# MiRaCLeXeoN/sduss

Hardware: AMD Instinct MI355X
Metric: images/sec (node), SDXL 1024^2 50-step, fixed prompt, CFG (higher is better)
Workload: dtype bf16; 1 GPU; SDXL-base-1.0 UNet 1024x1024 50-step Euler, CFG 5.0, 4 requests/step (denoiser batch 8) per GPU, is_sliced=False, random-init weights of the real architecture (2.57 B params), one data-parallel replica per GPU, no collective; resolution=1024, steps_per_image=50

## Files before the change

### include/mxdenoise.h

```cpp
#ifndef MXDENOISE_H
#define MXDENOISE_H

#include <stddef.h>
#include <stdint.h>

#ifdef __cplusplus
extern "C" {
#endif

enum { MX_F32 = 0, MX_F16 = 1, MX_BF16 = 2 };

const char* mx_last_error(void);
int mx_version(void);
#define MX_PROF_KINDS 12
int mx_profile_enable(int on);
int mx_profile_collect(double* out);
int mx_profile_records(double* out, int max_records);

size_t mx_groupnorm_halo_workspace_bytes(int N, int C, int cpg);
int mx_groupnorm_halo(void* stream, const void* x, const void* gamma, const void* beta, void* y,
                      int N, int C, int H, int W, int cpg, double eps, int padding,
                      const int32_t* latent_offset, int n_latents, const int32_t* patch_map,
                      const int32_t* padding_idx, int dtype, void* workspace);
int mx_halo_only(void* stream, const void* x, void* y, int N, int C, int H, int W,
// ... 89 lines not shown
#define MX_STATS_PITCH(slabs) (((slabs) + 3) & ~3)
int mx_row_stats(void* stream, const void* x, int ldx, float* stats, int M, int C);
int mx_conv3x3(void* stream, const mx_gemm_desc* d);
int mx_gemm_splitk(const mx_gemm_desc* d, int conv);
void mx_gemm_release_scratch(void* stream, int all);

#define MX_VT_POS(key) (((key) & ~12) | (((key) & 4) << 1) | (((key) & 8) >> 1))
#define MX_VT_LD(Lk) (((Lk) + 15) / 16 * 16)

int mx_attention(void* stream, const void* q, int ldq, const void* k, int ldk, const void* vt, int ldvt,
                 int64_t vt_batch_stride, void* o, int ldo, int B, int H, int Lq, int Lk, float scale);
#define MX_ATTN_QSCALE(scale) ((scale) * 1.4426950408889634f)
int mx_attention_prescaled(void* stream, const void* q, int ldq, const void* k, int ldk, const void* vt, int ldvt,
                           int64_t vt_batch_stride, void* o, int ldo, int B, int H, int Lq, int Lk);
int mx_attention_cross_prescaled(void* stream, const void* q, int ldq, const void* k, int ldk, const void* vt, int ldvt,
                                 int64_t vt_batch_stride, void* o, int ldo, int B, int H, int Lq, int Lk);
typedef struct mx_attn_problem {
  const void* q; const void* k; const void* vt; void* o;
  int64_t vt_batch_stride;
  int B, Lq, Lk, ldvt;
} mx_attn_problem;
int mx_attention_prescaled_grouped(void* stream, const mx_attn_problem* probs, int n, int ldq, int ldk, int ldo, int H);
int mx_attention_prescaled_bias(void* stream, const void* q, int ldq, const void* k, int ldk, const void* vt, int ldvt,
                                int64_t vt_batch_stride, void* o, int ldo, int B, int H, int Lq, int Lk, const float* bias, int ldb);
int mx_attention_prescaled_causal(void* stream, const void* q, int ldq, const void* k, int ldk, const void* vt, int ldvt,
                                  int64_t vt_batch_stride, void* o, int ldo, int B, int H, int L);

int mx_layernorm(void* stream, const void* x, void* y, const float* gamma, const float* beta,
                 int M, int C, float eps);

int mx_rmsnorm(void* stream, const void* x, void* y, const float* w, int M, int C, float eps);

int mx_layernorm_mod(void* stream, const void* x, void* y, void* y2, const float* scale, const float* shift,
                     const float* scale2, const float* shift2, int ldmod, int M, int C, int rows_per_batch, float eps);
int mx_layernorm_mod_grouped(void* stream, const void* x, void* y, void* y2, const float* scale, const float* shift, const float* scale2,
                             const float* shift2, int ldmod, int C, float eps, const int* batches, const int* rows_per_batch, int n);
int mx_rmsnorm_heads(void* stream, void* x, int ld, int nbatch, int rows_per_batch, int batch_rows, int row_off,
                     int heads_total, int heads_q, const float* wq, const float* wk, float eps, float q_scale);

size_t mx_groupnorm_nhwc_workspace_bytes(int B, int H, int W, int C);
int mx_groupnorm_nhwc(void* stream, const void* x, void* y, const float* gamma, const float* beta,
                      int B, int H, int W, int C, int groups, float eps, int silu, int patch,
                      void* workspace);

int mx_groupnorm_nhwc_cat(void* stream, const void* x, int C1, const void* x2, void* y, const float* gamma, const float* beta,
                          int B, int H, int W, int C, int groups, float eps, int silu, int patch, void* workspace);
int mx_groupnorm_nhwc_from_partials(void* stream, const void* x, void* y, const float* gamma, const float* beta, int B, int H, int W, int C, int groups, float eps,
                                    int silu, const float* part, int chunk, const float* add_bias, const float* add_rowbias, int ldrb, void* workspace);

typedef struct mx_gn_problem { const void* x; const void* x2; void* y; int B, H, W; } mx_gn_problem;
size_t mx_groupnorm_nhwc_grouped_workspace_bytes(const mx_gn_problem* probs, int n, int C);
int mx_groupnorm_nhwc_grouped(void* stream, const mx_gn_problem* probs, int n, int C1, const float* gamma, const float* beta, int C, int groups,
                              float eps, int silu, int patch, void* workspace);

typedef struct mx_unet_config {
  int in_channels, out_channels;
  int n_levels;
  int block_out_channels[4];
  int layers_per_block;
  int down_has_attn[4];
  int transformer_layers[4];
  int num_heads[4];
  int cross_attention_dim;
  int addition_time_embed_dim;
  int projection_class_embeddings_input_dim;
  int norm_num_groups;
  float norm_eps, transformer_norm_eps, layer_norm_eps;
} mx_unet_config;

typedef struct mx_weight_entry {
  const char* name;
  uint64_t offset;
  uint64_t bytes;
} mx_weight_entry;

typedef struct mx_unet mx_unet;

mx_unet* mx_unet_create(const mx_unet_config* cfg);
void mx_unet_destroy(mx_unet* u);
int mx_unet_set_weights(mx_unet* u, const void* blob, uint64_t blob_bytes,
                        const mx_weight_entry* table, int n_entries);
int mx_unet_set_context_key(mx_unet* u, uint64_t key);
int mx_unet_context_stats(const mx_unet* u, long* hits, long* misses);
size_t mx_unet_workspace_bytes(const mx_unet* u, int batch, int H, int W, int ctx_len);
int mx_unet_validate(const mx_unet* u, int batch, int H, int W, int ctx_len);
int mx_unet_forward(mx_unet* u, void* stream, const void* latents, int io_dtype, const float* timesteps,
                    const void* ehs, const void* text_embeds, const float* time_ids, void* out,
                    int batch, int H, int W, int ctx_len, int gn_patch, void* workspace, size_t workspace_bytes);
typedef struct mx_unet_group { const void* latents; void* out; int batch, H, W; } mx_unet_group;
size_t mx_unet_workspace_bytes_mixed(const mx_unet* u, const mx_unet_group* groups, int n_groups, int ctx_len);
int mx_unet_forward_mixed(mx_unet* u, void* stream, const mx_unet_group* groups, int n_groups, int io_dtype, const float* timesteps,
                          const void* ehs, const void* text_embeds, const float* time_ids, int ctx_len, int gn_patch, void* workspace,
                          size_t workspace_bytes);
int mx_unet_forward_mixed_trace(mx_unet* u, void* stream, const mx_unet_group* groups, int n_groups, int io_dtype, const float* timesteps,
                                const void* ehs, const void* text_embeds, const float* time_ids, int ctx_len, int gn_patch, void* workspace,
                                size_t workspace_bytes, const char* stage, void* stage_out, size_t stage_out_bytes);
int mx_unet_forward_trace(mx_unet* u, void* stream, const void* latents, int io_dtype, const float* timesteps,
                          const void* ehs, const void* text_embeds, const float* time_ids, void* out,
                          int batch, int H, int W, int ctx_len, int gn_patch, void* workspace,
                          size_t workspace_bytes, const char* stage, void* stage_out, size_t stage_out_bytes);

typedef int (*mx_allgather_fn)(void* ctx, void* stream, const void* send, void* recv, size_t bytes_per_rank);
typedef struct mx_pp_comm { int rank, world; mx_allgather_fn all_gather; void* ctx; } mx_pp_comm;
size_t mx_unet_workspace_bytes_pp(const mx_unet* u, int batch, int H_local, int W, int ctx_len, int world);
int mx_unet_forward_pp(mx_unet* u, void* stream, const void* latents_local, int io_dtype, const float* timesteps, const void* ehs,
                       const void* text_embeds, const float* time_ids, void* out_local, int batch, int H_local, int W, int ctx_len,
// ... 209 lines not shown
```

### sduss_amd/csrc/norm.hip

```cpp
#include <cstdlib>

#include "common.h"
#include "../../include/mxdenoise.h"

namespace mx {

struct GnGeom {
  int B, H, W, C;
  int tpr;
  int L;
  int th, tw;
  int tiles_y, tiles_x;
  const bf16_t* x2;
  int C1;
};

struct GnProb {
  GnGeom g;
  const bf16_t* x; bf16_t* y;
  float* part; float* coef;
  float* gpart;
  long y_img;
  int ppb;
  int patch;
};
struct GnGroup {
  GnProb p[MX_MAX_SEGS];
  int blk0[MX_MAX_SEGS + 1];
  int n;
};
__device__ __forceinline__ const GnProb& gn_locate(const GnGroup& G, int& local) {
  local = blockIdx.x;
  int s = 0;
#pragma unroll
  for (int i = 1; i < MX_MAX_SEGS; ++i) if (i < G.n && local >= G.blk0[i]) s = i;
  local -= G.blk0[s];
  return G.p[s];
}

__device__ __forceinline__ const bf16_t* gn_src(const bf16_t* x, const GnGeom& g, long pix, int ch) {
  if (g.x2 == nullptr) return x + pix * g.C + ch;
  return ch < g.C1 ? x + pix * g.C1 + ch : g.x2 + pix * (g.C - g.C1) + (ch - g.C1);
}

__global__ void gn_stats_kernel(const GnGroup G, const int groups) {
  extern __shared__ __attribute__((aligned(16))) float red[];
  const int t = threadIdx.x;
  int local;
  const GnProb& P = gn_locate(G, local);
  const GnGeom& g = P.g;
  const bf16_t* __restrict__ x = P.x;
  float* __restrict__ part = P.part;
  const int ntl = g.tiles_y * g.tiles_x;
  const int b = local / ntl;
  const int tile = local - b * ntl;
  const int ty = tile / g.tiles_x, tx = tile - ty * g.tiles_x;
  const int cv = t % g.tpr;
  const int pl = t / g.tpr;
  float s[8], ss[8];
#pragma unroll
  for (int e = 0; e < 8; ++e) { s[e] = 0.f; ss[e] = 0.f; }
  if (pl < g.L) {
    const int npix = g.th * g.tw;
    for (int pi = pl; pi < npix; pi += g.L) {
      const int py = pi / g.tw, px = pi - py * g.tw;
      const long pix = ((long)b * g.H + ty * g.th + py) * g.W + tx * g.tw + px;
      const u32x4 v = *reinterpret_cast<const u32x4*>(gn_src(x, g, pix, cv * 8));
#pragma unroll
      for (int e = 0; e < 4; ++e) {
        const float lo = bf16lo_to_f32(v[e]), hi = bf16hi_to_f32(v[e]);
        s[2 * e] += lo; ss[2 * e] += lo * lo;
        s[2 * e + 1] += hi; ss[2 * e + 1] += hi * hi;
      }
    }
#pragma unroll
    for (int e = 0; e < 8; ++e) {
      red[((long)pl * g.C + cv * 8 + e) * 2] = s[e];
      red[((long)pl * g.C + cv * 8 + e) * 2 + 1] = ss[e];
    }
  }
  __syncthreads();
  float* __restrict__ gpart = P.gpart;
  float* chs = red + (long)g.L * g.C * 2;
  for (int c = t; c < g.C; c += blockDim.x) {
    float a = 0.f, q = 0.f;
    for (int l = 0; l < g.L; ++l) { a += red[((long)l * g.C + c) * 2]; q += red[((long)l * g.C + c) * 2 + 1]; }
    if (gpart != nullptr) { chs[2 * c] = a; chs[2 * c + 1] = q; continue; }
    float* dst = part + (((long)b * (g.tiles_y * g.tiles_x) + tile) * g.C + c) * 2;
    dst[0] = a; dst[1] = q;
  }
  if (gpart != nullptr) {
// ... 107 lines not shown
      double s = 0.0, q = 0.0;
      for (int tl = sub; tl < ntl; tl += 8) {
        const float2 v = *reinterpret_cast<const float2*>(gp + ((long)tl * groups + gi) * 2);
        s += (double)v.x; q += (double)v.y;
      }
      fsub[gi][sub][0] = s; fsub[gi][sub][1] = q;
    }
    __syncthreads();
    const int cpg = g.C / groups;
    const double cnt = (double)g.H * g.W * cpg;
    for (int gi = t; gi < groups; gi += blockDim.x) {
      double s = 0.0, q = 0.0;
#pragma unroll
      for (int sub = 0; sub < 8; ++sub) { s += fsub[gi][sub][0]; q += fsub[gi][sub][1]; }
      const double mean = s / cnt;
      double var = q / cnt - mean * mean;
      if (var < 0.0) var = 0.0;
      mr[gi][0] = mean;
      mr[gi][1] = 1.0 / sqrt(var + (double)eps);
    }
    __syncthreads();
    if (pl >= g.L) return;
#pragma unroll
    for (int e = 0; e < 8; ++e) {
      const int ch = cv * 8 + e;
      const int gi = ch / cpg;
      const double rg = mr[gi][1] * (double)gamma[ch];
      sc[e] = (float)rg;
      sf[e] = (float)((double)beta[ch] - rg * mr[gi][0]);
    }
  } else {
    if (pl >= g.L) return;
    const float* cf = coef + ((long)b * g.C + cv * 8) * 2;
#pragma unroll
    for (int e = 0; e < 8; ++e) { sc[e] = cf[2 * e]; sf[e] = cf[2 * e + 1]; }
  }
  const int hw = g.H * g.W;
  const int p0 = pblk * pix_per_block;
  const int p1 = min(p0 + pix_per_block, hw);
  for (int pi = p0 + pl; pi < p1; pi += g.L) {
    const u32x4 v = *reinterpret_cast<const u32x4*>(gn_src(x, g, (long)b * hw + pi, cv * 8));
    u32x4 o;
#pragma unroll
    for (int e = 0; e < 4; ++e) {
      float lo = bf16lo_to_f32(v[e]) * sc[2 * e] + sf[2 * e];
      float hi = bf16hi_to_f32(v[e]) * sc[2 * e + 1] + sf[2 * e + 1];
      if (SILU) { lo = silu_f(lo); hi = silu_f(hi); }
      o[e] = pack_bf16x2(lo, hi);
    }
    *reinterpret_cast<u32x4*>(y + (long)b * y_img + (long)pi * g.C + cv * 8) = o;
  }
}

__global__ __launch_bounds__(64) void gn_pp_sums_kernel(const float* __restrict__ part, double* __restrict__ sums, GnGeom g, int groups) {
  const int grp = blockIdx.x, b = blockIdx.y, lane = threadIdx.x;
  const int cpg = g.C / groups;
  const int ntiles = g.tiles_y * g.tiles_x;
  double s = 0.0, q = 0.0;
  for (int it = lane; it < ntiles * cpg; it += 64) {
    const int tile = it / cpg, c = it - tile * cpg;
    const float* src = part + (((long)b * ntiles + tile) * g.C + grp * cpg + c) * 2;
    s += (double)src[0];
    q += (double)src[1];
  }
  s = wave_sum_d(s);
  q = wave_sum_d(q);
  if (lane == 0) { sums[((long)b * groups + grp) * 2] = s; sums[((long)b * groups + grp) * 2 + 1] = q; }
}

__global__ __launch_bounds__(64) void gn_pp_coef_kernel(const double* __restrict__ all_sums, const float* __restrict__ gamma,
                                                        const float* __restrict__ beta, float* __restrict__ coef, int B, int C,
                                                        int groups, int world, double cnt, float eps,
                                                        const double* __restrict__ fresh_own, int own_rank) {
  const int grp = blockIdx.x, b = blockIdx.y, lane = threadIdx.x;
  const int cpg = C / groups;
  double s = 0.0, q = 0.0;
  for (int r = 0; r < world; ++r) {
    s += all_sums[(((long)r * B + b) * groups + grp) * 2];
    q += all_sums[(((long)r * B + b) * groups + grp) * 2 + 1];
  }
  double var_fallback = 0.0;
  if (fresh_own) {
    const long o = (((long)own_rank * B + b) * groups + grp) * 2, f = ((long)b * groups + grp) * 2;
    s += (double)world * (fresh_own[f] - all_sums[o]);
    q += (double)world * (fresh_own[f + 1] - all_sums[o + 1]);
    const double lc = cnt / world, lm = fresh_own[f] / lc;
    var_fallback = fresh_own[f + 1] / lc - lm * lm;
    if (var_fallback < 0.0) var_fallback = 0.0;
  }
  const double mean = s / cnt;
  double var = q / cnt - mean * mean;
  if (var < 0.0) var = var_fallback;
  const double rstd = 1.0 / sqrt(var + (double)eps);
  for (int c = lane; c < cpg; c += 64) {
    const int ch = grp * cpg + c;
    coef[((long)b * C + ch) * 2] = (float)(rstd * (double)gamma[ch]);
    coef[((long)b * C + ch) * 2 + 1] = (float)((double)beta[ch] - rstd * (double)gamma[ch] * mean);
  }
}

static int gn_geom(GnGeom& g, int B, int H, int W, int C, int patch) {
  MX_CHECK(C % 8 == 0 && C / 8 <= 1024, "groupnorm: C must be a multiple of 8 and <= 8192");
  g.B = B; g.H = H; g.W = W; g.C = C;
  g.x2 = nullptr; g.C1 = C;
  g.tpr = C / 8;
  g.L = 1024 / g.tpr;
// ... 32 lines not shown
  return mx_groupnorm_nhwc_cat(stream, x, C, nullptr, y, gamma, beta, B, H, W, C, groups, eps, silu, patch, workspace);
}

namespace mx {
static size_t gn_fill(GnGroup& G, int i, const void* x, int C1, const void* x2, void* y, long y_img, int B, int H, int W, int C, int patch, char* ws) {
  GnProb& P = G.p[i];
  if (patch >= H && patch >= W) patch = 0;
  if (patch != 0 && patch < 2) { set_error("groupnorm: patch must be 0 or >= 2"); return 0; }
  if (gn_geom(P.g, B, H, W, C, patch)) return 0;
  if (x2) { P.g.x2 = (const bf16_t*)x2; P.g.C1 = C1; }
  const size_t ntiles = (size_t)P.g.tiles_y * P.g.tiles_x;
  P.x = (const bf16_t*)x; P.y = (bf16_t*)y; P.y_img = y_img; P.patch = patch;
  P.part = (float*)ws;
  P.gpart = nullptr;
  P.coef = P.part + (size_t)B * ntiles * C * 2;
  const int hw = H * W;
  P.ppb = P.g.L * 8 > hw ? hw : P.g.L * 8;
  return (((size_t)B * ntiles * C * 2 + (size_t)B * C * 2) * sizeof(float) + 255) & ~(size_t)255;
}
static void gn_prefix(GnGroup& G, int which, int groups) {
  long t = 0;
  for (int i = 0; i < G.n; ++i) {
    G.blk0[i] = (int)t;
    const GnGeom& g = G.p[i].g;
    t += which == 0 ? (long)g.B * g.tiles_y * g.tiles_x : which == 1 ? (long)g.B * groups : (long)g.B * cdiv(g.H * g.W, G.p[i].ppb);
  }
  for (int i = G.n; i <= MX_MAX_SEGS; ++i) G.blk0[i] = (int)t;
}
static int gn_launch_stats(hipStream_t s, GnGroup& G, int C, int groups = 0) {
  const GnGeom& g = G.p[0].g;
  const int threads = ((g.tpr * g.L + 63) / 64) * 64;
  const size_t smem = ((size_t)g.L * C * 2 + (groups > 0 ? (size_t)C * 2 : 0)) * sizeof(float);
  MX_CHECK(smem <= 160 * 1024, "groupnorm: LDS budget exceeded");
  gn_prefix(G, 0, 0);
  hipLaunchKernelGGL(gn_stats_kernel, dim3(G.blk0[MX_MAX_SEGS]), dim3(threads), smem, s, G, groups);
  MX_LAUNCH_CHECK();
  return 0;
}
static int gn_launch_apply(hipStream_t s, GnGroup& G, int silu, bool fold = false, const float* gamma = nullptr, const float* beta = nullptr, int groups = 0, float eps = 0.f) {
  const GnGeom& g = G.p[0].g;
  const int threads = ((g.tpr * g.L + 63) / 64) * 64;
  gn_prefix(G, 2, 0);
  const dim3 grid(G.blk0[MX_MAX_SEGS]), block(threads);
  if (fold) {
    if (silu) hipLaunchKernelGGL((gn_apply_kernel<true, true>), grid, block, 0, s, G, gamma, beta, groups, eps);
    else hipLaunchKernelGGL((gn_apply_kernel<false, true>), grid, block, 0, s, G, gamma, beta, groups, eps);
  } else {
    if (silu) hipLaunchKernelGGL((gn_apply_kernel<true, false>), grid, block, 0, s, G, gamma, beta, groups, eps);
    else hipLaunchKernelGGL((gn_apply_kernel<false, false>), grid, block, 0, s, G, gamma, beta, groups, eps);
  }
  MX_LAUNCH_CHECK();
  return 0;
}
}

extern "C" size_t mx_groupnorm_nhwc_grouped_workspace_bytes(const mx_gn_problem* probs, int n, int C) {
  size_t t = 0;
  for (int i = 0; probs && i < n; ++i) t += mx_groupnorm_nhwc_workspace_bytes(probs[i].B, probs[i].H, probs[i].W, C);
  return t;
}

extern "C" int mx_groupnorm_nhwc_grouped(void* stream, const mx_gn_problem* probs, int n, int C1, const float* gamma, const float* beta, int C,
                                         int groups, float eps, int silu, int patch, void* workspace) {
  using namespace mx;
  MX_CHECK(probs && n >= 1 && n <= MX_MAX_SEGS && gamma && beta && workspace, "groupnorm: grouped launch needs 1..MX_MAX_SEGS problems and its operands");
  MX_CHECK(groups > 0 && C % groups == 0, "groupnorm: C % groups != 0");
  if (patch > 0 && groups <= kFoldGroups && n > 1) {
    mx_gn_problem ex[MX_MAX_SEGS], sl[MX_MAX_SEGS];
    int ne = 0, ns = 0;
    for (int i = 0; i < n; ++i) {
      if (patch >= probs[i].H && patch >= probs[i].W) ex[ne++] = probs[i]; else sl[ns++] = probs[i];
    }
    if (ne > 0 && ns > 0) {
      if (mx_groupnorm_nhwc_grouped(stream, ex, ne, C1, gamma, beta, C, groups, eps, silu, patch, workspace)) return 1;
      return mx_groupnorm_nhwc_grouped(stream, sl, ns, C1, gamma, beta, C, groups, eps, silu, patch,
                                       (char*)workspace + mx_groupnorm_nhwc_grouped_workspace_bytes(ex, ne, C));
    }
  }
  GnGroup G;
  G.n = n;
  char* ws = (char*)workspace;
  double bytes = 0;
  for (int i = 0; i < n; ++i) {
    const mx_gn_problem& q = probs[i];
    MX_CHECK(q.x && q.y && q.B > 0 && q.H > 0 && q.W > 0, "groupnorm: null operand / empty problem");
    MX_CHECK(q.x2 == nullptr || (C1 > 0 && C1 < C && C1 % 8 == 0 && (C - C1) % 8 == 0), "groupnorm: bad channel split");
    MX_CHECK((q.x2 != nullptr) == (probs[0].x2 != nullptr), "groupnorm: grouped launch: either every problem reads a channel concatenation or none");
    const size_t used = gn_fill(G, i, q.x, C1, q.x2, q.y, (long)q.H * q.W * C, q.B, q.H, q.W, C, patch, ws);
    if (!used) return 1;
    MX_CHECK(used <= mx_groupnorm_nhwc_workspace_bytes(q.B, q.H, q.W, C), "groupnorm: internal workspace bound exceeded");
    ws += mx_groupnorm_nhwc_workspace_bytes(q.B, q.H, q.W, C);
    bytes += 3.0 * 2.0 * q.B * q.H * (double)q.W * C;
  }
  hipStream_t s = (hipStream_t)stream;
  prof_begin(s, PROF_NORM, 0.0, bytes);
  bool fold = groups <= kFoldGroups;
  for (int i = 0; i < n; ++i) fold = fold && G.p[i].patch == 0;
  if (fold) {
    for (int i = 0; i < n; ++i) G.p[i].gpart = G.p[i].part;
    if (gn_launch_stats(s, G, C, groups)) return 1;
    if (gn_launch_apply(s, G, silu, true, gamma, beta, groups, eps)) return 1;
    prof_end(s);
    return 0;
  }
  if (gn_launch_stats(s, G, C)) return 1;
  gn_prefix(G, 1, groups);
  hipLaunchKernelGGL(gn_fold_kernel, dim3(G.blk0[MX_MAX_SEGS]), dim3(kFoldThreads), 0, s, G, gamma, beta, groups, eps);
  MX_LAUNCH_CHECK();
  if (gn_launch_apply(s, G, silu)) return 1;
  prof_end(s);
  return 0;
}

extern "C" int mx_groupnorm_nhwc_cat(void* stream, const void* x, int C1, const void* x2, void* y, const float* gamma, const float* beta,
                                     int B, int H, int W, int C, int groups, float eps, int silu, int patch,
                                     void* workspace) {
  mx_gn_problem q;
  q.x = x; q.x2 = x2; q.y = y; q.B = B; q.H = H; q.W = W;
  return mx_groupnorm_nhwc_grouped(stream, &q, 1, C1, gamma, beta, C, groups, eps, silu, patch, workspace);
}

extern "C" int mx_groupnorm_nhwc_from_partials(void* stream, const void* x, void* y, const float* gamma, const float* beta, int B, int H, int W, int C, int groups,
                                               float eps, int silu, const float* part, int chunk, const float* add_bias, const float* add_rowbias, int ldrb,
                                               void* workspace) {
  using namespace mx;
  MX_CHECK(x && y && gamma && beta && part && workspace && B > 0 && H > 0 && W > 0, "groupnorm: null operand / empty problem");
  MX_CHECK(groups > 0 && C % groups == 0 && chunk > 0 && (H * W) % chunk == 0 && ((uintptr_t)part & 15) == 0, "groupnorm: bad groups / chunk / alignment");
  GnGroup G;
  G.n = 1;
  if (!gn_fill(G, 0, x, C, nullptr, y, (long)H * W * C, B, H, W, C, 0, (char*)workspace)) return 1;
  GnGroup F = G;
  F.p[0].part = const_cast<float*>(part);
  F.p[0].g.tiles_y = H * W / chunk; F.p[0].g.tiles_x = 1; F.p[0].g.th = chunk; F.p[0].g.tw = 1;
  hipStream_t s = (hipStream_t)stream;
  prof_begin(s, PROF_NORM, 0.0, 2.0 * 2.0 * B * H * (double)W * C);
  gn_prefix(F, 1, groups);
  MX_CHECK(add_rowbias == nullptr || (add_bias != nullptr && ldrb >= C), "groupnorm: add_rowbias needs add_bias and ldrb >= C");
  hipLaunchKernelGGL(gn_fold_kernel, dim3(F.blk0[MX_MAX_SEGS]), dim3(kFoldThreads), 0, s, F, gamma, beta, groups, eps, add_bias, add_rowbias, ldrb);
  MX_LAUNCH_CHECK();
  if (gn_launch_apply(s, G, silu)) return 1;
  prof_end(s);
  return 0;
}

namespace mx {
int launch_gn_pp_partial(hipStream_t s, const void* x, int C1, const void* x2, int B, int H, int W, int C, int groups, void* workspace, double* sums) {
  GnGroup G;
// ... 356 lines not shown
```

### sduss_amd/csrc/unet_sdxl.cpp

```cpp
#include <hip/hip_runtime.h>

#include <algorithm>
#include <cstring>
#include <functional>
#include <map>
#include <string>
#include <vector>

#include "../../include/mxdenoise.h"
#include "common.h"
#include "graph_cache.h"
#include "patch_cache.h"
#include "plan_base.h"

namespace mx {
int launch_prep_latent(hipStream_t s, const void* in, int dtype, void* out, int B, int Cin, int HW, int CP);
int launch_nhwc_to_nchw(hipStream_t s, const void* in, void* out, int dtype, int B, int C, int HW, int ld);
int launch_time_embed(hipStream_t s, const float* timesteps, const void* text_embeds, const float* time_ids,
                      void* tsin, void* addin, int B, int d0, int text_dim, int da);
int launch_concat(hipStream_t s, const void* a, const void* b, void* out, long M, int C1, int C2);
size_t gn_workspace_exact(int B, int H, int W, int C, int patch);
int launch_sq_diff_partial(hipStream_t s, const void* a, const void* b, long elems_per_sample, int B, double* partial, const int* slot = nullptr);
int launch_gn_pp_partial(hipStream_t s, const void* x, int C1, const void* x2, int B, int H, int W, int C, int groups, void* workspace, double* sums);
int launch_gn_pp_finish(hipStream_t s, const void* x, int C1, const void* x2, void* y, long y_img_elems, const float* gamma, const float* beta, const double* all_sums,
// ... 293 lines not shown
    d.out_scale = l.out_scale;
    if (l.a2) { d.a2 = l.a2; d.lda2 = l.lda2; d.k_split = l.lda; }
    d.a = l.a; d.lda = l.lda; d.w = wb(l.stem + ".weight", (size_t)l.N * l.K); d.bias = wf(l.stem + ".bias", l.N);
    d.c = l.c; d.ldc = l.ldc; d.M = l.M; d.N = l.N; d.K = l.K; d.residual = l.residual; d.ldr = l.ldr; d.flags = l.flags;
    if (l.ln) use_ln(d, *l.ln, l.stem + ".colsum", l.ln_final);
    if (l.stats_out) return gemm_with_stats(d, *l.stats_out, l.finalise);
    return gemm(d, false);
  }
  int conv_cin_valid = 0;
  bool conv(const Conv& c) {
    const bf16_t* x = c.in.padded ? c.in.padded : c.in.t;
    const int Cin = c.Cin, Cout = c.Cout, stride = c.stride, up = c.up;
    mx_gemm_desc d; std::memset(&d, 0, sizeof(d));
    d.vhalo = c.in.padded ? 1 : 0;
    const int Hv = c.Hin << up, Wv = c.Win << up;
    d.a = x; d.w = wb(c.prefix + ".weight", (size_t)Cout * 9 * Cin); d.bias = wf(c.prefix + ".bias", Cout);
    d.c = c.out; d.ldc = Cout; d.B = gB[0]; d.Hin = c.Hin; d.Win = c.Win; d.Cin = Cin;
    d.Hout = (Hv + stride - 1) / stride; d.Wout = (Wv + stride - 1) / stride; d.stride = stride; d.up = up;
    d.corner_patch = c.corner_patch;
    d.M = gB[0] * d.Hout * d.Wout; d.N = Cout; d.K = 9 * Cin;
    d.rowbias = c.rowbias; d.ldrb = c.ldrb; d.rows_per_batch = d.Hout * d.Wout;
    d.residual = c.residual; d.ldr = Cout;
    mx_gemm_seg sg[MX_MAX_SEGS];
    if (ng > 1) {
      std::memset(sg, 0, sizeof(sg));
      long in0 = 0, out0 = 0;
      for (int g = 0; g < ng; ++g) {
        mx_gemm_seg& q = sg[g];
        q.B = gB[g]; q.Hin = ch[g]; q.Win = cw[g];
        q.Hout = ((ch[g] << up) + stride - 1) / stride; q.Wout = ((cw[g] << up) + stride - 1) / stride;
        q.M = gB[g] * q.Hout * q.Wout; q.rows_per_batch = q.Hout * q.Wout;
        q.a = x + in0 * Cin; q.c = c.out + out0 * Cout;
        q.residual = c.residual ? (const bf16_t*)c.residual + out0 * Cout : nullptr;
        q.rowbias = c.rowbias ? c.rowbias + (long)gb0[g] * c.ldrb : nullptr;
        in0 += (long)gB[g] * ch[g] * cw[g]; out0 += q.M;
      }
      d.segs = sg; d.n_segs = ng;
    }
    if (c.gn_part && c.gn_done && ng == 1 && mx_gemm_gn_partials_supported(&d, 1)) { d.gn_part_out = c.gn_part; *c.gn_done = true; }
    d.cin_valid = conv_cin_valid;
    return gemm(d, true);
  }
  bool groupnorm(const bf16_t* x, bf16_t* y, const std::string& prefix, int h, int wd, int C, float eps, bool silu, int patch,
                 const bf16_t* x2 = nullptr, int C1 = 0) {
    if (!ok()) return false;
    const size_t m = ar.mark();
    mx_gn_problem pr[MX_MAX_SEGS];
    long r0 = 0;
    for (int k = 0; k < ng; ++k) {
      pr[k].x = x + r0 * (x2 ? C1 : C); pr[k].x2 = x2 ? x2 + r0 * (C - C1) : nullptr; pr[k].y = y + r0 * C;
      pr[k].B = gB[k]; pr[k].H = ch[k]; pr[k].W = cw[k];
      r0 += (long)gB[k] * ch[k] * cw[k];
    }
    const size_t need = ng > 1 ? mx_groupnorm_nhwc_grouped_workspace_bytes(pr, ng, C) : mx::gn_workspace_exact(gB[0], h, wd, C, patch);
    void* ws = ar.alloc(need);
    if (!ws) return fail("workspace too small");
    const float* g = wf(prefix + ".weight", C); const float* b = wf(prefix + ".bias", C);
    if (ok() && !quiet()) {
      if (mx_groupnorm_nhwc_grouped(stream, pr, ng, x2 ? C1 : C, g, b, C, u->cfg.norm_num_groups, eps, silu ? 1 : 0, patch, ws))
        fail(std::string("groupnorm: ") + mx_last_error());
    }
    ar.release(m);
    return ok();
  }
  bool groupnorm_from_partials(const bf16_t* x, bf16_t* y, const std::string& prefix, int h, int wd, int C, float eps, bool silu, const float* part,
                               const float* add_bias, const float* add_rowbias, int ldrb) {
    if (!ok()) return false;
    const size_t m = ar.mark();
    void* ws = ar.alloc(mx::gn_workspace_exact(gB[0], h, wd, C, 0));
    if (!ws) return fail("workspace too small");
    const float* g = wf(prefix + ".weight", C); const float* b = wf(prefix + ".bias", C);
    if (ok() && !quiet()) {
      if (mx_groupnorm_nhwc_from_partials(stream, x, y, g, b, gB[0], h, wd, C, u->cfg.norm_num_groups, eps, silu ? 1 : 0, part, 64, add_bias, add_rowbias, ldrb, ws))
        fail(std::string("groupnorm: ") + mx_last_error());
    }
    ar.release(m);
    return ok();
  }
  bool attention(const bf16_t* q, int ldq, const bf16_t* k, int ldk, const bf16_t* vt, int ldvt, long vt_bstride, bf16_t* o,
                 int ldo, int heads, int Lq, int Lk) {
    if (!ok()) return false;
    if (quiet()) return true;
    if (mx_attention_prescaled(stream, q, ldq, k, ldk, vt, ldvt, vt_bstride, o, ldo, B, heads, Lq, Lk))
      return fail(std::string("attention: ") + mx_last_error());
    return true;
  }
  bool attention_grouped(const mx_attn_problem* pr, int ldq, int ldk, int ldo, int heads) {
    if (!ok()) return false;
    if (quiet()) return true;
    if (mx_attention_prescaled_grouped(stream, pr, ng, ldq, ldk, ldo, heads)) return fail(std::string("attention: ") + mx_last_error());
    return true;
  }
  int level_patch(int level) const { return gn_patch > 0 ? std::max(gn_patch >> level, 1) : 0; }

  ConvIn alloc_conv_in(int h, int wd, int C) {
    if (!is_pp()) return {alloc<bf16_t>((size_t)rows() * C), nullptr};
    bf16_t* P = alloc_padded(h, wd, C);
    return {interior(P, wd, C), P};
  }
  bool norm_into(const ConvIn& n, const bf16_t* x, const std::string& prefix, int h, int wd, int C, int level, const bf16_t* x2 = nullptr, int C1 = 0) {
    if (!is_pp()) return groupnorm(x, n.t, prefix, h, wd, C, u->cfg.norm_eps, true, level_patch(level), x2, C1);
    groupnorm_pp(x, n.t, (long)(h + 2) * wd * C, prefix, h, wd, C, u->cfg.norm_eps, true, level, x2, C1);
    return halo_exchange(n.padded, h, wd, C);
  }
  bool block_conv(Conv c, int level) {
    if (is_pp()) return conv(c);
    c.corner_patch = level_patch(level - c.up);
    return pc ? pc_conv(c, level) : conv(c);
  }
// ... 980 lines not shown
```

### sduss_amd/lib.py

```python
from __future__ import annotations

import ctypes as C
import os
from typing import Optional

_HERE = os.path.dirname(os.path.abspath(__file__))
LIB_PATH = os.path.join(_HERE, "libmxdenoise.so")

MX_F32, MX_F16, MX_BF16 = 0, 1, 2
EPI_SILU, EPI_GEGLU, EPI_OUT_F32, EPI_QKV, EPI_GELU_TANH, EPI_RES_BCAST, EPI_RMSNORM, EPI_GELU, EPI_QUICK_GELU, EPI_GEGLU_TANH = 1, 2, 4, 8, 16, 32, 64, 128, 256, 512


class MxError(RuntimeError):
    """Raised for every non-zero status of the C ABI (the reference's launcher only printed
    cudaGetLastError and went on -- norm_silu_concat.cu:434-437; SURVEY.md section 8b asks to raise)."""


MAX_SEGS = 4


class GemmSeg(C.Structure):
    _fields_ = [
        ("a", C.c_void_p), ("a2", C.c_void_p), ("c", C.c_void_p), ("residual", C.c_void_p), ("vt", C.c_void_p), ("rowbias", C.c_void_p),
        ("gate", C.c_void_p), ("ln_stats", C.c_void_p), ("stats_out", C.c_void_p),
# ... 109 lines not shown
    _fields_ = [("vocab_size", C.c_int), ("hidden_size", C.c_int), ("intermediate_size", C.c_int), ("num_hidden_layers", C.c_int),
                ("num_attention_heads", C.c_int), ("max_position_embeddings", C.c_int), ("hidden_act", C.c_int), ("projection_dim", C.c_int),
                ("eos_token_id", C.c_int), ("hidden_layer", C.c_int), ("layer_norm_eps", C.c_float)]


class T5ConfigC(C.Structure):
    _fields_ = [("vocab_size", C.c_int), ("d_model", C.c_int), ("d_ff", C.c_int), ("num_layers", C.c_int), ("num_heads", C.c_int),
                ("layer_norm_epsilon", C.c_float)]


class VAEConfigC(C.Structure):
    _fields_ = [("latent_channels", C.c_int), ("out_channels", C.c_int), ("n_levels", C.c_int), ("block_out_channels", C.c_int * 4),
                ("layers_per_block", C.c_int), ("norm_num_groups", C.c_int), ("norm_eps", C.c_float)]


IMAGE_RGB8_HWC, IMAGE_F32_CHW = 0, 1


class VAEEncodeArgs(C.Structure):
    _fields_ = [("image", C.c_void_p), ("image_format", C.c_int), ("posterior_noise", C.c_void_p), ("start_noise", C.c_void_p),
                ("keep", C.c_void_p), ("sigma", C.c_void_p), ("latents", C.c_void_p), ("io_dtype", C.c_int),
                ("scaling_factor", C.c_float), ("shift_factor", C.c_float)]


class WeightEntry(C.Structure):
    _fields_ = [("name", C.c_char_p), ("offset", C.c_uint64), ("bytes", C.c_uint64)]


_vp, _i, _f, _d, _i64, _sz = C.c_void_p, C.c_int, C.c_float, C.c_double, C.c_int64, C.c_size_t
SYMBOLS = {
    "mx_last_error": (C.c_char_p, []),
    "mx_version": (_i, []),
    "mx_profile_enable": (_i, [_i]),
    "mx_profile_collect": (_i, [C.POINTER(C.c_double)]),
    "mx_profile_records": (_i, [C.POINTER(C.c_double), _i]),
    "mx_groupnorm_halo_workspace_bytes": (_sz, [_i, _i, _i]),
    "mx_groupnorm_halo": (_i, [_vp, _vp, _vp, _vp, _vp, _i, _i, _i, _i, _i, _d, _i, _vp, _i, _vp, _vp, _i, _vp]),
    "mx_halo_only": (_i, [_vp, _vp, _vp, _i, _i, _i, _i, _vp, _i]),
    "mx_gemm": (_i, [_vp, C.POINTER(GemmDesc)]),
    "mx_conv3x3": (_i, [_vp, C.POINTER(GemmDesc)]),
    "mx_gemm_stats_slabs": (_i, [C.POINTER(GemmDesc)]),
    "mx_gemm_ln_prefers_pass": (_i, [C.POINTER(GemmDesc)]),
    "mx_row_stats": (_i, [_vp, _vp, _i, _vp, _i, _i]),
    "mx_attention": (_i, [_vp, _vp, _i, _vp, _i, _vp, _i, _i64, _vp, _i, _i, _i, _i, _i, _f]),
    "mx_attention_prescaled": (_i, [_vp, _vp, _i, _vp, _i, _vp, _i, _i64, _vp, _i, _i, _i, _i, _i]),
    "mx_attention_cross_prescaled": (_i, [_vp, _vp, _i, _vp, _i, _vp, _i, _i64, _vp, _i, _i, _i, _i, _i]),
    "mx_layernorm": (_i, [_vp, _vp, _vp, _vp, _vp, _i, _i, _f]),
    "mx_groupnorm_nhwc_workspace_bytes": (_sz, [_i, _i, _i, _i]),
    "mx_groupnorm_nhwc": (_i, [_vp, _vp, _vp, _vp, _vp, _i, _i, _i, _i, _i, _f, _i, _i, _vp]),
    "mx_groupnorm_nhwc_cat": (_i, [_vp, _vp, _i, _vp, _vp, _vp, _vp, _i, _i, _i, _i, _i, _f, _i, _i, _vp]),
    "mx_attention_prescaled_grouped": (_i, [_vp, C.POINTER(AttnProblem), _i, _i, _i, _i, _i]),
    "mx_groupnorm_nhwc_grouped_workspace_bytes": (_sz, [C.POINTER(GnProblem), _i, _i]),
    "mx_groupnorm_nhwc_grouped": (_i, [_vp, C.POINTER(GnProblem), _i, _i, _vp, _vp, _i, _i, _f, _i, _i, _vp]),
    "mx_unet_workspace_bytes_mixed": (_sz, [_vp, C.POINTER(UNetGroup), _i, _i]),
    "mx_unet_forward_mixed": (_i, [_vp, _vp, C.POINTER(UNetGroup), _i, _i, _vp, _vp, _vp, _vp, _i, _i, _vp, _sz]),
    "mx_unet_forward_mixed_trace": (_i, [_vp, _vp, C.POINTER(UNetGroup), _i, _i, _vp, _vp, _vp, _vp, _i, _i, _vp, _sz, C.c_char_p, _vp, _sz]),
    "mx_mmdit_workspace_bytes_mixed": (_sz, [_vp, C.POINTER(UNetGroup), _i, _i]),
    "mx_mmdit_forward_mixed": (_i, [_vp, _vp, C.POINTER(UNetGroup), _i, _i, _vp, _vp, _vp, _i, _vp, _sz]),
    "mx_unet_create": (_vp, [C.POINTER(UNetConfigC)]),
    "mx_unet_destroy": (None, [_vp]),
    "mx_unet_set_context_key": (_i, [_vp, C.c_uint64]),
    "mx_unet_context_stats": (_i, [_vp, C.POINTER(C.c_long), C.POINTER(C.c_long)]),
    "mx_unet_set_weights": (_i, [_vp, _vp, C.c_uint64, C.POINTER(WeightEntry), _i]),
    "mx_unet_workspace_bytes": (_sz, [_vp, _i, _i, _i, _i]),
    "mx_unet_validate": (_i, [_vp, _i, _i, _i, _i]),
    "mx_unet_forward": (_i, [_vp, _vp, _vp, _i, _vp, _vp, _vp, _vp, _vp, _i, _i, _i, _i, _i, _vp, _sz]),
    "mx_forest_predict": (_i, [_vp, _vp, _vp, _vp, _vp, _vp, _i, _vp, _i, _i, _vp]),
    "mx_skip_counters_bytes": (_sz, [_i, _i, _i]),
    "mx_skip_decide_host": (_i, [C.POINTER(DeviceForestC), _i, _i, _i, _i, _vp, _vp, _vp, _vp, _vp, _vp, _vp, _vp, _vp]),
    "mx_skip_decide_device": (_i, [_vp, C.POINTER(SkipDecideArgs)]),
    "mx_mmdit_workspace_bytes_pp": (_sz, [_vp, _i, _i, _i, _i, _i]),
    "mx_mmdit_pp_state_bytes": (_sz, [_vp, _i, _i, _i, _i, _i]),
    "mx_mmdit_forward_pp": (_i, [_vp, _vp, _vp, _i, _vp, _vp, _vp, _vp, _i, _i, _i, _i, _vp, _vp, _vp, _sz]),
    "mx_mmdit_pp_comm_plan": (_i, [_vp, _i, _i, _i, _i, _vp]),
    "mx_unet_pp_state_bytes": (_sz, [_vp, _i, _i, _i, _i, _i]),
    "mx_unet_forward_pp_stale": (_i, [_vp, _vp, _vp, _i, _vp, _vp, _vp, _vp, _vp, _i, _i, _i, _i, _vp, _vp, _vp, _sz]),
    "mx_unet_block_cache_bytes": (_sz, [_vp, _i, _i, _i]),
    "mx_gemm_splitk": (_i, [_vp, _i]),
    "mx_gemm_release_scratch": (None, [_vp, _i]),
    "mx_gemm_ln_final_supported": (_i, [C.POINTER(GemmDesc)]),
    "mx_gemm_launches": (_i, [C.POINTER(GemmDesc)]),
    "mx_gemm_gn_partials_supported": (_i, [C.POINTER(GemmDesc), _i]),
    "mx_gemm_form": (_i, [C.POINTER(GemmDesc), _i]),
    "mx_gemm_kernel_name": (_i, [C.POINTER(GemmDesc), _i, _i, C.c_char_p, _i]),
    "mx_gemm_kernel_names": (_i, [C.c_char_p, _i]),
    "mx_attention_kernel_name": (_i, [_i, _i, _i, _i, _i, _i, _i, _i, _i, _i, C.c_char_p, _i]),
    "mx_attention_kernel_names": (_i, [C.c_char_p, _i]),
    "mx_groupnorm_nhwc_from_partials": (_i, [_vp, _vp, _vp, _vp, _vp, _i, _i, _i, _i, _i, C.c_float, _i, _vp, _i, _vp, _vp, _i, _vp]),
    "mx_unet_patch_cache_bytes": (_sz, [_vp, _i, _i, _i, _i]),
    "mx_mmdit_patch_cache_bytes": (_sz, [_vp, _i, _i, _i, _i, _i]),
    "mx_mmdit_workspace_bytes_cached_mixed": (_sz, [_vp, C.POINTER(UNetGroup), _i, _i, _i]),
    "mx_mmdit_forward_cached_mixed": (_i, [_vp, _vp, C.POINTER(UNetGroup), _i, _i, _vp, _vp, _vp, _i, _i, _vp, _sz, _vp]),
    "mx_unet_workspace_bytes_cached_mixed": (_sz, [_vp, C.POINTER(UNetGroup), _i, _i, _i]),
    "mx_unet_forward_cached_mixed": (_i, [_vp, _vp, C.POINTER(UNetGroup), _i, _i, _vp, _vp, _vp, _vp, _i, _i, _vp, _sz, _vp]),
    "mx_unet_forward_cached": (_i, [_vp, _vp, _vp, _i, _vp, _vp, _vp, _vp, _vp, _i, _i, _i, _i, _i, _vp, _sz, _vp]),
    "mx_mmdit_block_cache_bytes": (_sz, [_vp, _i, _i, _i, _i]),
    "mx_mmdit_forward_cached": (_i, [_vp, _vp, _vp, _i, _vp, _vp, _vp, _vp, _i, _i, _i, _i, _vp, _sz, _vp]),
    "mx_unet_forward_trace": (_i, [_vp, _vp, _vp, _i, _vp, _vp, _vp, _vp, _vp, _i, _i, _i, _i, _i, _vp, _sz,
                                   C.c_char_p, _vp, _sz]),
    "mx_unet_workspace_bytes_pp": (_sz, [_vp, _i, _i, _i, _i, _i]),
    "mx_unet_forward_pp": (_i, [_vp, _vp, _vp, _i, _vp, _vp, _vp, _vp, _vp, _i, _i, _i, _i, C.POINTER(PPComm), _vp, _sz]),
    "mx_unet_pp_comm_plan": (_i, [_vp, _i, _i, _i, _i, C.POINTER(PPComm)]),
    "mx_attention_prescaled_chunked": (_i, [_vp, _vp, _i, _vp, _i, _vp, _i, _i64, _vp, _i, _i, _i, _i, _i, _i, _i64, _i64, _i64]),
    "mx_layernorm_mod": (_i, [_vp, _vp, _vp, _vp, _vp, _vp, _vp, _vp, _i, _i, _i, _i, _f]),
    "mx_layernorm_mod_grouped": (_i, [_vp, _vp, _vp, _vp, _vp, _vp, _vp, _vp, _i, _i, _f, _vp, _vp, _i]),
    "mx_rmsnorm_heads": (_i, [_vp, _vp, _i, _i, _i, _i, _i, _i, _i, _vp, _vp, _f, _f]),
# ... 118 lines not shown
```

Baseline: 1.517 images/s.

## Add register-resident one-pass GroupNorm kernel for small-slab NHWC shapes

Adds a one-pass GroupNorm kernel for NHWC tensors. Each 1024-thread block loads one (image, group) slab into registers, reduces mean and variance in double precision, then applies the affine transform and optional SiLU straight from registers. This replaces the stats/partials/apply chain with a single launch that reads the input once, for group widths and spatial sizes whose slab fits a register cap (SDXL's 64x64 and 32x32 levels). Workspace is only allocated for problems that still use the chain. The risks are high register pressure at 1024 threads per block, and the eligibility check depends on having at least half as many slabs as there are CUs.

```diff
diff --git a/include/mxdenoise.h b/include/mxdenoise.h
--- a/include/mxdenoise.h
+++ b/include/mxdenoise.h
@@ -165,6 +165,8 @@
 size_t mx_groupnorm_nhwc_grouped_workspace_bytes(const mx_gn_problem* probs, int n, int C);
 int mx_groupnorm_nhwc_grouped(void* stream, const mx_gn_problem* probs, int n, int C1, const float* gamma, const float* beta, int C, int groups,
                               float eps, int silu, int patch, void* workspace);
+enum { MX_GN_FORM_CHAIN = 0, MX_GN_FORM_ONE_PASS = 1 };
+int mx_groupnorm_nhwc_form(int B, int H, int W, int C, int groups, int C1, int patch, int producer_stats);
 
 typedef struct mx_unet_config {
   int in_channels, out_channels;
diff --git a/sduss_amd/csrc/norm.hip b/sduss_amd/csrc/norm.hip
--- a/sduss_amd/csrc/norm.hip
+++ b/sduss_amd/csrc/norm.hip
@@ -29,14 +29,15 @@
   int blk0[MX_MAX_SEGS + 1];
   int n;
 };
-__device__ __forceinline__ const GnProb& gn_locate(const GnGroup& G, int& local) {
-  local = blockIdx.x;
+__device__ __forceinline__ const GnProb& gn_locate_at(const GnGroup& G, int idx, int& local) {
+  local = idx;
   int s = 0;
 #pragma unroll
   for (int i = 1; i < MX_MAX_SEGS; ++i) if (i < G.n && local >= G.blk0[i]) s = i;
   local -= G.blk0[s];
   return G.p[s];
 }
+__device__ __forceinline__ const GnProb& gn_locate(const GnGroup& G, int& local) { return gn_locate_at(G, blockIdx.x, local); }
 
 __device__ __forceinline__ const bf16_t* gn_src(const bf16_t* x, const GnGeom& g, long pix, int ch) {
   if (g.x2 == nullptr) return x + pix * g.C + ch;
@@ -250,6 +251,121 @@
   }
 }
 
+constexpr int kOnePassThreads = 1024;
+constexpr int kOnePassDataRegs = 64;
+constexpr size_t kOnePassSlabCap = 240 * 1024;
+
+template <int NW> struct GnWords;
+template <> struct GnWords<4> { typedef u32x4 type; };
+template <> struct GnWords<2> { typedef u32x2 type; };
+template <> struct GnWords<1> { typedef unsigned type; };
+template <int NW> __device__ __forceinline__ unsigned gn_word(const typename GnWords<NW>::type& v, int e) {
+  if constexpr (NW == 1) return v; else return v[e];
+}
+template <int NW> __device__ __forceinline__ void gn_set_word(typename GnWords<NW>::type& v, int e, unsigned w) {
+  if constexpr (NW == 1) v = w; else v[e] = w;
+}
+
+template <int NW, int K>
+__device__ __forceinline__ void gn_slab_load(typename GnWords<NW>::type (&v)[K], const char* __restrict__ base, unsigned off0, unsigned stride, unsigned last) {
+#pragma unroll
+  for (int k = 0; k < K; ++k) v[k] = *reinterpret_cast<const typename GnWords<NW>::type*>(base + (size_t)min(off0 + (unsigned)k * stride, last));
+}
+
+template <int CPG, int K, bool SILU>
+__global__ __launch_bounds__(kOnePassThreads) void gn_one_pass_kernel(const GnGroup G, const float* __restrict__ gamma, const float* __restrict__ beta,
+                                                                      const int groups, const float eps) {
+  constexpr int NW = CPG % 8 == 0 ? 4 : CPG % 4 == 0 ? 2 : 1;
+  constexpr int NV = CPG / (2 * NW);
+  constexpr int TL = kOnePassThreads / NV;
+  typedef typename GnWords<NW>::type vec_t;
+  const int t = threadIdx.x;
+  const int n = gridDim.x, xr = blockIdx.x & 7;
+  const int slab = xr * (n >> 3) + min(xr, n & 7) + (blockIdx.x >> 3);
+  int local;
+  const GnProb& P = gn_locate_at(G, slab, local);
+  const GnGeom& g = P.g;
+  const int b = local / groups;
+  const int grp = local - b * groups;
+  const int hw = g.H * g.W;
+  const int vl = t % NV;
+  const int tl = t / NV < TL ? t / NV : hw;
+  const int ch = grp * CPG + vl * (2 * NW);
+  vec_t v[K];
+  if (g.x2 == nullptr || ch < g.C1) {
+    const int ld = g.x2 == nullptr ? g.C : g.C1;
+    gn_slab_load<NW, K>(v, reinterpret_cast<const char*>(P.x + (long)b * hw * ld), (unsigned)(tl * ld + ch) * 2u, (unsigned)(TL * ld) * 2u,
+                        (unsigned)((hw - 1) * ld + ch) * 2u);
+  } else {
+    const int ld = g.C - g.C1, c2 = ch - g.C1;
+    gn_slab_load<NW, K>(v, reinterpret_cast<const char*>(g.x2 + (long)b * hw * ld), (unsigned)(tl * ld + c2) * 2u, (unsigned)(TL * ld) * 2u,
+                        (unsigned)((hw - 1) * ld + c2) * 2u);
+  }
+  float ga[2 * NW], be[2 * NW];
+#pragma unroll
+  for (int e = 0; e < 2 * NW; ++e) { ga[e] = gamma[ch + e]; be[e] = beta[ch + e]; }
+  float s = 0.f, q = 0.f;
+#pragma unroll
+  for (int k = 0; k < K; ++k) {
+    if (tl + k * TL < hw) {
+#pragma unroll
+      for (int e = 0; e < NW; ++e) {
+        const unsigned w = gn_word<NW>(v[k], e);
+        const float lo = bf16lo_to_f32(w), hi = bf16hi_to_f32(w);
+        s += lo; q += lo * lo;
+        s += hi; q += hi * hi;
+      }
+    }
+  }
+#pragma unroll
+  for (int k = 0; k < K; ++k) {
+#pragma unroll
+    for (int e = 0; e < NW; ++e) {
+      unsigned w = gn_word<NW>(v[k], e);
+      asm volatile("" : "+v"(w));
+      gn_set_word<NW>(v[k], e, w);
+    }
+  }
+  __shared__ double wsum[kOnePassThreads / 64][2];
+  double ds = wave_sum_d((double)s), dq = wave_sum_d((double)q);
+  if ((t & 63) == 0) { wsum[t >> 6][0] = ds; wsum[t >> 6][1] = dq; }
+  __syncthreads();
+  ds = 0.0; dq = 0.0;
+#pragma unroll
+  for (int w = 0; w < kOnePassThreads / 64; ++w) { ds += wsum[w][0]; dq += wsum[w][1]; }
+  const double cnt = (double)hw * CPG;
+  const double mean = ds / cnt;
+  double var = dq / cnt - mean * mean;
+  if (var < 0.0) var = 0.0;
+  const double rstd = 1.0 / sqrt(var + (double)eps);
+  float sc[2 * NW], sf[2 * NW];
+#pragma unroll
+  for (int e = 0; e < 2 * NW; ++e) {
+    const double rg = rstd * (double)ga[e];
+    sc[e] = (float)rg;
+    sf[e] = (float)((double)be[e] - rg * mean);
+  }
+  char* __restrict__ y = reinterpret_cast<char*>(P.y + (long)b * P.y_img);
+  int tla = tl;
+  asm volatile("" : "+v"(tla));
+  const unsigned yoff = (unsigned)(tla * g.C + ch) * 2u, ystride = (unsigned)(TL * g.C) * 2u;
+#pragma unroll
+  for (int k = 0; k < K; ++k) {
+    if (tla + k * TL < hw) {
+      vec_t o;
+#pragma unroll
+      for (int e = 0; e < NW; ++e) {
+        const unsigned w = gn_word<NW>(v[k], e);
+        float lo = bf16lo_to_f32(w) * sc[2 * e] + sf[2 * e];
+        float hi = bf16hi_to_f32(w) * sc[2 * e + 1] + sf[2 * e + 1];
+        if (SILU) { lo = silu_f(lo); hi = silu_f(hi); }
+        gn_set_word<NW>(o, e, pack_bf16x2(lo, hi));
+      }
+      *reinterpret_cast<vec_t*>(y + (size_t)(yoff + (unsigned)k * ystride)) = o;
+    }
+  }
+}
+
 __global__ __launch_bounds__(64) void gn_pp_sums_kernel(const float* __restrict__ part, double* __restrict__ sums, GnGeom g, int groups) {
   const int grp = blockIdx.x, b = blockIdx.y, lane = threadIdx.x;
   const int cpg = g.C / groups;
@@ -388,6 +504,65 @@
   MX_LAUNCH_CHECK();
   return 0;
 }
+
+static int gn_one_pass_words(int cpg) { return cpg % 8 == 0 ? 4 : cpg % 4 == 0 ? 2 : 1; }
+static int gn_one_pass_regs(int cpg) { return gn_one_pass_words(cpg) == 1 ? kOnePassDataRegs / 2 : kOnePassDataRegs; }
+static int gn_one_pass_k(int hw, int cpg) {
+  const int nw = gn_one_pass_words(cpg);
+  return cdiv(hw, kOnePassThreads / (cpg / (2 * nw)));
+}
+static bool gn_one_pass_eligible(int B, int H, int W, int C, int groups, int C1) {
+  if (groups <= 0 || C % groups != 0 || B <= 0 || H <= 0 || W <= 0) return false;
+  const int cpg = C / groups;
+  if (cpg != 10 && cpg != 20 && cpg != 30 && cpg != 40 && cpg != 60 && cpg != 80) return false;
+  if (C1 % 8 != 0 || (C - C1) % 8 != 0) return false;
+  const long hw = (long)H * W;
+  if ((size_t)hw * cpg * 2 > kOnePassSlabCap) return false;
+  if (gn_one_pass_k((int)hw, cpg) * gn_one_pass_words(cpg) > gn_one_pass_regs(cpg)) return false;
+  return 2L * B * groups >= cu_count();
+}
+
+template <int CPG, int NW>
+static void gn_one_pass_pick(hipStream_t s, const GnGroup& G, int kneed, int silu, const float* gamma, const float* beta, int groups, float eps) {
+  const dim3 grid(G.blk0[MX_MAX_SEGS]), block(kOnePassThreads);
+  constexpr int K0 = kOnePassDataRegs / 4 / NW, K1 = kOnePassDataRegs / 2 / NW, K2 = kOnePassDataRegs / NW;
+#define MX_GN1(KK)                                                                                                       \
+  do {                                                                                                                   \
+    if (silu) hipLaunchKernelGGL((gn_one_pass_kernel<CPG, KK, true>), grid, block, 0, s, G, gamma, beta, groups, eps);   \
+    else hipLaunchKernelGGL((gn_one_pass_kernel<CPG, KK, false>), grid, block, 0, s, G, gamma, beta, groups, eps);       \
+  } while (0)
+  if (kneed <= K0) MX_GN1(K0);
+  else if (kneed <= K1) MX_GN1(K1);
+  else if constexpr (NW > 1) MX_GN1(K2);
+#undef MX_GN1
+}
+static int gn_launch_one_pass(hipStream_t s, GnGroup& G, int C, int silu, const float* gamma, const float* beta, int groups, float eps) {
+  const int cpg = C / groups;
+  int kneed = 1;
+  for (int i = 0; i < G.n; ++i) {
+    const int k = gn_one_pass_k(G.p[i].g.H * G.p[i].g.W, cpg);
+    if (k > kneed) kneed = k;
+  }
+  MX_CHECK(kneed * gn_one_pass_words(cpg) <= gn_one_pass_regs(cpg), "groupnorm: one-pass form on a slab past its cap");
+  gn_prefix(G, 1, groups);
+  switch (cpg) {
+    case 10: gn_one_pass_pick<10, 1>(s, G, kneed, silu, gamma, beta, groups, eps); break;
+    case 20: gn_one_pass_pick<20, 2>(s, G, kneed, silu, gamma, beta, groups, eps); break;
+    case 30: gn_one_pass_pick<30, 1>(s, G, kneed, silu, gamma, beta, groups, eps); break;
+    case 40: gn_one_pass_pick<40, 4>(s, G, kneed, silu, gamma, beta, groups, eps); break;
+    case 60: gn_one_pass_pick<60, 2>(s, G, kneed, silu, gamma, beta, groups, eps); break;
+    case 80: gn_one_pass_pick<80, 4>(s, G, kneed, silu, gamma, beta, groups, eps); break;
+    default: MX_CHECK(false, "groupnorm: one-pass form is not built for this group width");
+  }
+  MX_LAUNCH_CHECK();
+  return 0;
+}
+}
+
+extern "C" int mx_groupnorm_nhwc_form(int B, int H, int W, int C, int groups, int C1, int patch, int producer_stats) {
+  if (producer_stats) return MX_GN_FORM_CHAIN;
+  if (patch > 0 && !(patch >= H && patch >= W)) return MX_GN_FORM_CHAIN;
+  return mx::gn_one_pass_eligible(B, H, W, C, groups, C1 > 0 ? C1 : C) ? MX_GN_FORM_ONE_PASS : MX_GN_FORM_CHAIN;
 }
 
 extern "C" size_t mx_groupnorm_nhwc_grouped_workspace_bytes(const mx_gn_problem* probs, int n, int C) {
@@ -399,7 +574,7 @@
 extern "C" int mx_groupnorm_nhwc_grouped(void* stream, const mx_gn_problem* probs, int n, int C1, const float* gamma, const float* beta, int C,
                                          int groups, float eps, int silu, int patch, void* workspace) {
   using namespace mx;
-  MX_CHECK(probs && n >= 1 && n <= MX_MAX_SEGS && gamma && beta && workspace, "groupnorm: grouped launch needs 1..MX_MAX_SEGS problems and its operands");
+  MX_CHECK(probs && n >= 1 && n <= MX_MAX_SEGS && gamma && beta, "groupnorm: grouped launch needs 1..MX_MAX_SEGS problems and its operands");
   MX_CHECK(groups > 0 && C % groups == 0, "groupnorm: C % groups != 0");
   if (patch > 0 && groups <= kFoldGroups && n > 1) {
     mx_gn_problem ex[MX_MAX_SEGS], sl[MX_MAX_SEGS];
@@ -413,22 +588,50 @@
                                        (char*)workspace + mx_groupnorm_nhwc_grouped_workspace_bytes(ex, ne, C));
     }
   }
+  for (int i = 0; i < n; ++i) {
+    const mx_gn_problem& q = probs[i];
+    MX_CHECK(q.x && q.y && q.B > 0 && q.H > 0 && q.W > 0, "groupnorm: null operand / empty problem");
+    MX_CHECK(q.x2 == nullptr || (C1 > 0 && C1 < C && C1 % 8 == 0 && (C - C1) % 8 == 0), "groupnorm: bad channel split");
+    MX_CHECK((q.x2 != nullptr) == (probs[0].x2 != nullptr), "groupnorm: grouped launch: either every problem reads a channel concatenation or none");
+  }
+  hipStream_t s = (hipStream_t)stream;
+  mx_gn_problem chain[MX_MAX_SEGS];
+  {
+    GnGroup O;
+    O.n = 0;
+    int nchain = 0;
+    double obytes = 0;
+    for (int i = 0; i < n; ++i) {
+      const mx_gn_problem& q = probs[i];
+      if (mx_groupnorm_nhwc_form(q.B, q.H, q.W, C, groups, q.x2 ? C1 : 0, patch, 0) != MX_GN_FORM_ONE_PASS) { chain[nchain++] = q; continue; }
+      GnProb& P = O.p[O.n++];
+      P = GnProb{};
+      P.g.B = q.B; P.g.H = q.H; P.g.W = q.W; P.g.C = C;
+      P.g.x2 = (const bf16_t*)q.x2; P.g.C1 = q.x2 ? C1 : C;
+      P.x = (const bf16_t*)q.x; P.y = (bf16_t*)q.y; P.y_img = (long)q.H * q.W * C;
+      obytes += 2.0 * 2.0 * q.B * q.H * (double)q.W * C;
+    }
+    if (O.n > 0) {
+      prof_begin(s, PROF_NORM, 0.0, obytes);
+      if (gn_launch_one_pass(s, O, C, silu, gamma, beta, groups, eps)) return 1;
+      prof_end(s);
+      if (nchain == 0) return 0;
+      probs = chain; n = nchain;
+    }
+  }
+  MX_CHECK(workspace, "groupnorm: the stats / fold / apply chain needs its workspace");
   GnGroup G;
   G.n = n;
   char* ws = (char*)workspace;
   double bytes = 0;
   for (int i = 0; i < n; ++i) {
     const mx_gn_problem& q = probs[i];
-    MX_CHECK(q.x && q.y && q.B > 0 && q.H > 0 && q.W > 0, "groupnorm: null operand / empty problem");
-    MX_CHECK(q.x2 == nullptr || (C1 > 0 && C1 < C && C1 % 8 == 0 && (C - C1) % 8 == 0), "groupnorm: bad channel split");
-    MX_CHECK((q.x2 != nullptr) == (probs[0].x2 != nullptr), "groupnorm: grouped launch: either every problem reads a channel concatenation or none");
     const size_t used = gn_fill(G, i, q.x, C1, q.x2, q.y, (long)q.H * q.W * C, q.B, q.H, q.W, C, patch, ws);
     if (!used) return 1;
     MX_CHECK(used <= mx_groupnorm_nhwc_workspace_bytes(q.B, q.H, q.W, C), "groupnorm: internal workspace bound exceeded");
     ws += mx_groupnorm_nhwc_workspace_bytes(q.B, q.H, q.W, C);
     bytes += 3.0 * 2.0 * q.B * q.H * (double)q.W * C;
   }
-  hipStream_t s = (hipStream_t)stream;
   prof_begin(s, PROF_NORM, 0.0, bytes);
   bool fold = groups <= kFoldGroups;
   for (int i = 0; i < n; ++i) fold = fold && G.p[i].patch == 0;
diff --git a/sduss_amd/csrc/unet_sdxl.cpp b/sduss_amd/csrc/unet_sdxl.cpp
--- a/sduss_amd/csrc/unet_sdxl.cpp
+++ b/sduss_amd/csrc/unet_sdxl.cpp
@@ -369,9 +369,18 @@
       pr[k].B = gB[k]; pr[k].H = ch[k]; pr[k].W = cw[k];
       r0 += (long)gB[k] * ch[k] * cw[k];
     }
-    const size_t need = ng > 1 ? mx_groupnorm_nhwc_grouped_workspace_bytes(pr, ng, C) : mx::gn_workspace_exact(gB[0], h, wd, C, patch);
-    void* ws = ar.alloc(need);
-    if (!ws) return fail("workspace too small");
+    size_t need = 0;
+    if (ng > 1) {
+      mx_gn_problem chain[MX_MAX_SEGS];
+      int nc = 0;
+      for (int k = 0; k < ng; ++k)
+        if (patch > 0 || mx_groupnorm_nhwc_form(pr[k].B, pr[k].H, pr[k].W, C, u->cfg.norm_num_groups, x2 ? C1 : 0, 0, 0) == MX_GN_FORM_CHAIN) chain[nc++] = pr[k];
+      need = mx_groupnorm_nhwc_grouped_workspace_bytes(chain, nc, C);
+    } else if (mx_groupnorm_nhwc_form(gB[0], h, wd, C, u->cfg.norm_num_groups, x2 ? C1 : 0, patch, 0) == MX_GN_FORM_CHAIN) {
+      need = mx::gn_workspace_exact(gB[0], h, wd, C, patch);
+    }
+    void* ws = need ? ar.alloc(need) : nullptr;
+    if (need && !ws) return fail("workspace too small");
     const float* g = wf(prefix + ".weight", C); const float* b = wf(prefix + ".bias", C);
     if (ok() && !quiet()) {
       if (mx_groupnorm_nhwc_grouped(stream, pr, ng, x2 ? C1 : C, g, b, C, u->cfg.norm_num_groups, eps, silu ? 1 : 0, patch, ws))
diff --git a/sduss_amd/lib.py b/sduss_amd/lib.py
--- a/sduss_amd/lib.py
+++ b/sduss_amd/lib.py
@@ -185,6 +185,7 @@
     "mx_attention_prescaled_grouped": (_i, [_vp, C.POINTER(AttnProblem), _i, _i, _i, _i, _i]),
     "mx_groupnorm_nhwc_grouped_workspace_bytes": (_sz, [C.POINTER(GnProblem), _i, _i]),
     "mx_groupnorm_nhwc_grouped": (_i, [_vp, C.POINTER(GnProblem), _i, _i, _vp, _vp, _i, _i, _f, _i, _i, _vp]),
+    "mx_groupnorm_nhwc_form": (_i, [_i, _i, _i, _i, _i, _i, _i, _i]),
     "mx_unet_workspace_bytes_mixed": (_sz, [_vp, C.POINTER(UNetGroup), _i, _i]),
     "mx_unet_forward_mixed": (_i, [_vp, _vp, C.POINTER(UNetGroup), _i, _i, _vp, _vp, _vp, _vp, _i, _i, _vp, _sz]),
     "mx_unet_forward_mixed_trace": (_i, [_vp, _vp, C.POINTER(UNetGroup), _i, _i, _vp, _vp, _vp, _vp, _i, _i, _vp, _sz, C.c_char_p, _vp, _sz]),
```

Result: no change. 1.523 images/s, median of 6 (+0.4%).
